# jeremy29tien/robosuite-benchmark

Hardware: AMD Instinct MI355X
Metric: SAC grad-steps/sec (batch=256, 1e6 buffer) at 1/2/4/8 GPU (higher is better)
Workload: dtype f32

## Files before the change

### robosuite_benchmark_amd/csrc/sac_trainer.hip

```cpp
#include "sac_common.h"

#include <algorithm>
#include <cmath>
#include <cstdlib>
#include <chrono>
#include <cstring>
#include <mutex>
#include <vector>

namespace sac {

typedef float f32x4 __attribute__((ext_vector_type(4)));

constexpr int H = 256;
constexpr float LOG_SIG_MAX = 2.0f, LOG_SIG_MIN = -20.0f, TANH_EPS = 1e-6f;
constexpr float ADAM_B1 = 0.9f, ADAM_B2 = 0.999f, ADAM_EPS = 1e-8f;
constexpr float ADAM_1MB1 = (float)(1.0 - 0.9), ADAM_1MB2 = (float)(1.0 - 0.999);
constexpr int DIAG_TRACE_CAP = 4096;
constexpr int M_SAC = 0, M_TD3_CRITIC = 1, M_TD3_ACTOR = 2;
constexpr int RD = 4;

struct StepArg {
    long long step_now;
    long long adam_t;
// ... 47 lines not shown
    float *diag_dev;
    const float *eps1, *eps2;
};

struct DwLayer {
    const float *dYT, *XT;
    long long xt_off;
    float *P, *PT, *MT, *VT, *G;
    float *bias, *mb, *vb, *gb;
    float *TP, *Tbias;
    int N, K, ldp, ldt, nk, job0, xt_from_slot;
    float lr;
    int k_base, pad_;
};
constexpr int NDW = 12;
struct DwTable {
    const DwLayer *L;
    int job0[NDW];
    int njobs;
    const unsigned *abort;
};

#ifdef SAC_STAMPS
__device__ unsigned long long g_stamps[5 * 512 * 16];
#define STAMP(kid, i)                                                                              \
    do {                                                                                           \
        __builtin_amdgcn_sched_barrier(0);                                                         \
        if (threadIdx.x == 0 && blockIdx.x < 512) {                                                \
            g_stamps[((kid) * 512 + blockIdx.x) * 16 + (i)] = wall_clock64();                      \
        }                                                                                          \
        __builtin_amdgcn_sched_barrier(0);                                                         \
    } while (0)
#define STAMP_CLK(kid, i)                                                                          \
    do {                                                                                           \
        if (threadIdx.x == 0 && blockIdx.x < 512) g_stamps[((kid) * 512 + blockIdx.x) * 16 + (i)] = clock64(); \
    } while (0)
#else
#define STAMP(kid, i) do { } while (0)
#define STAMP_CLK(kid, i) do { } while (0)
#endif

__device__ __forceinline__ int lds_off(int row, int k, int KL) {
    return row * KL + ((((k >> 2) ^ (row & 15)) << 2) | (k & 3));
}
#define SB() __builtin_amdgcn_sched_barrier(0)
#define USE_FROM_HERE(x) asm volatile("" : "+v"(x))
__device__ __forceinline__ void lds_barrier() { asm volatile("s_waitcnt lgkmcnt(0)\n\ts_barrier" ::: "memory"); }
template <typename T>
__device__ __forceinline__ T sload(const T *p) {
    return *(const __attribute__((address_space(4))) T *)(uintptr_t)p;
}
__device__ __forceinline__ f32x4 ld4(const float *p) { return *reinterpret_cast<const f32x4 *>(p); }
__device__ __forceinline__ float ld1g(const float *p) { return *(const __attribute__((address_space(1))) float *)(uintptr_t)p; }
__device__ __forceinline__ void st1g(float *p, float v) {
    __hip_atomic_store((__attribute__((address_space(1))) float *)(uintptr_t)p, v, __ATOMIC_RELAXED, __HIP_MEMORY_SCOPE_AGENT);
}

template <int NBYTES>
__device__ __forceinline__ void kernarg_prefetch() {
    typedef const __attribute__((address_space(4))) int *kptr;
    kptr ka = (kptr)__builtin_amdgcn_kernarg_segment_ptr();
    constexpr int NL = (NBYTES + 63) / 64;
    static_assert(NL <= 16, "kernarg_prefetch: more than 16 lines");
    int x[16];
#pragma unroll
    for (int i = 0; i < 16; ++i) x[i] = ka[i < NL ? i * 16 : 0];
    asm volatile("" ::"s"(x[0]), "s"(x[1]), "s"(x[2]), "s"(x[3]), "s"(x[4]), "s"(x[5]), "s"(x[6]), "s"(x[7]), "s"(x[8]),
                 "s"(x[9]), "s"(x[10]), "s"(x[11]), "s"(x[12]), "s"(x[13]), "s"(x[14]), "s"(x[15]));
}

__device__ __forceinline__ AlphaStep alpha_step(const Ctl *ctl, const float *part_logpi, int NB, int B, float target_entropy,
                                                float lr, int auto_alpha, double bc1, double bc2s) {
    AlphaStep r;
    const float la = sload(&ctl->log_alpha), m0 = sload(&ctl->a_m), v0 = sload(&ctl->a_v);
    if (!auto_alpha) { r.alpha = 1.0f; r.alpha_loss = 0.0f; r.log_alpha = la; r.m = m0; r.v = v0; return r; }
    float sum = 0.f;
    for (int i = 0; i < NB; ++i) sum += sload(part_logpi + i);
    const float mean_lp = sum / (float)B + target_entropy;
    r.alpha_loss = -((la * mean_lp) + 0.0f);
    const float gr = -mean_lp;
    r.m = m0 + ADAM_1MB1 * (gr - m0);
    r.v = v0 * ADAM_B2 + ADAM_1MB2 * gr * gr;
    const float step_size = (float)((double)lr / bc1);
    const float denom = sqrtf(r.v) / (float)bc2s + 1e-8f;
    r.log_alpha = la + (-step_size * r.m) / denom;
    r.alpha = expf(r.log_alpha);
    return r;
}
__device__ __forceinline__ void st4(float *p, f32x4 v) { *reinterpret_cast<f32x4 *>(p) = v; }

template <int NT, int D = RD>
struct WRing {
    f32x4 b[D][NT];
    const float *wp[NT];
    __device__ __forceinline__ void init(const float *W, int ldw, int n_base, int n_stride, int s_off = 0) {
        const int lane = threadIdx.x & 63;
#pragma unroll
        for (int t = 0; t < NT; ++t)
            wp[t] = W + ((size_t)((n_base + t * n_stride) >> 4) * (ldw >> 4) + s_off) * 256 + 4 * lane;
    }
    __device__ __forceinline__ void fill_part(int KS, int u0, int u1, int lo = 0) {
#pragma unroll
        for (int u = 0; u < D; ++u)
            if (u >= u0 && u < u1 && u < KS && u >= lo) {
#pragma unroll
                for (int t = 0; t < NT; ++t) b[u][t] = ld4(wp[t] + 256 * u);
// ... 912 lines not shown
    }
#pragma unroll
    for (int o = 32; o > 0; o >>= 1) {
#pragma unroll
        for (int q = 0; q < NS; ++q) {
            sm[q] += __shfl_xor(sm[q], o); sq[q] += __shfl_xor(sq[q], o);
            mx[q] = fmaxf(mx[q], __shfl_xor(mx[q], o)); mn[q] = fminf(mn[q], __shfl_xor(mn[q], o));
        }
        lsum += __shfl_xor(lsum, o);
    }
    double *sh = reinterpret_cast<double *>(red);
    if (lane == 0) {
#pragma unroll
        for (int q = 0; q < NS; ++q) {
            sh[wave * 32 + q] = sm[q]; sh[wave * 32 + 6 + q] = sq[q]; sh[wave * 32 + 12 + q] = mx[q]; sh[wave * 32 + 18 + q] = mn[q];
        }
        sh[wave * 32 + 24] = lsum;
    }
    lds_barrier();
    float *const dlast = d.diag_dev;
    auto put = [&](int di, float v) {
        dlast[di] = v;
        if (loop_pos == 0) d.diag_first[di] = v;
        if (loop_pos < DIAG_TRACE_CAP) d.diag_trace[(size_t)loop_pos * SAC_DIAG_N + di] = v;
    };
    if (threadIdx.x < NS) {
        const int q = threadIdx.x;
        if ((q < 5) ? (sa.pad & 1) : (sa.pad & 2)) {
            double s = 0, s2 = 0, MX = -INFINITY, MN = INFINITY;
            for (int w = 0; w < 4; ++w) {
                s += sh[w * 32 + q]; s2 += sh[w * 32 + 6 + q];
                MX = fmax(MX, sh[w * 32 + 12 + q]); MN = fmin(MN, sh[w * 32 + 18 + q]);
            }
            const double cnt = (q < 5) ? (double)B : (double)B * d.A;
            const double mean = s / cnt;
            double var = s2 / cnt - mean * mean;
            if (var < 0) var = 0;
            const int base = (q < 3) ? SAC_D_Q1_MEAN + 4 * q : SAC_D_LOGPI_MEAN + 4 * (q - 3);
            put(base, (float)mean); put(base + 1, (float)sqrt(var)); put(base + 2, (float)MX); put(base + 3, (float)MN);
            if (q == 3) put(SAC_D_QF1_LOSS, (float)mean);
            if (q == 4) put(SAC_D_QF2_LOSS, (float)mean);
        }
    } else if (threadIdx.x == 64 && (sa.pad & 2)) {
        double s = 0;
        for (int w = 0; w < 4; ++w) s += sh[w * 32 + 24];
        put(SAC_D_POLICY_LOSS, (float)(-s / B));
    }
    if (sa.pad2 & 2u) {
        __syncthreads();
        if (threadIdx.x < SAC_DIAG_N) d.diag_last[threadIdx.x] = ld_sc1(d.diag_dev + threadIdx.x);
    }
}

__device__ __forceinline__ void dw_adam_body(const Dev &d, const DwTable &T, const float *__restrict__ S, const StepArg &sa,
                                             float *red, float *redb, float *trs, int vblock, unsigned aborted) {
    const int B = d.B;
    const int wave = threadIdx.x >> 6, lane = threadIdx.x & 63;
    const int r = lane & 15, g = lane >> 4;
    const Ctl *cp = d.ctl;
    float *const dlast = (sa.pad2 & 2u) ? d.diag_last : d.diag_dev;
    const bool keep_grad = (sa.pad2 & 2u) != 0;
    const int jb = vblock - 1;
    if (jb >= 0) {
        STAMP(4 - 2 * (sa.loop_pos & 1), 0);
        int li = 0;
#pragma unroll
        for (int q = 1; q < NDW; ++q) li = (jb >= T.job0[q]) ? q : li;
        union { DwLayer J; unsigned long long w[sizeof(DwLayer) / 8]; } ud;
        {
            const __attribute__((address_space(4))) unsigned long long *src =
                (const __attribute__((address_space(4))) unsigned long long *)(uintptr_t)(T.L + li);
#pragma unroll
            for (int q = 0; q < (int)(sizeof(DwLayer) / 8); ++q) ud.w[q] = src[q];
        }
        const DwLayer &J = ud.J;
#ifdef SAC_STAMPS
        { unsigned long long probe = ud.w[0]; asm volatile("" :: "s"(probe)); }
        STAMP(4, 3);
#endif
        const int jj = jb - J.job0;
        const int n0 = 16 * (jj / J.nk), k0 = J.k_base + 64 * (jj % J.nk);
        const int k_own = k0 + 16 * wave + r;
        const bool own_valid = k_own < J.K;
        const size_t ot = frag_off(k_own, n0 + 4 * g, J.ldt);
        const size_t tile_floats = (size_t)(B >> 4) * 256;
        const float *XT = (J.xt_from_slot ? S + J.xt_off : J.XT) + (size_t)(k0 >> 4) * tile_floats;
        const float *YT = J.dYT + (size_t)(n0 >> 4) * tile_floats;
        const int per = (B / 16) / 4;
        const int rem = (B / 16) - 4 * per;
        const int s0 = wave * per + (wave < rem ? wave : rem);
        const int s1 = s0 + per + (wave < rem ? 1 : 0);
        const float *yp = YT + 4 * lane;
        const float *xp = XT + 4 * lane;
        f32x4 acc[4] = {};
        float bsum = 0.f;
        const f32x4 zero4 = {0.f, 0.f, 0.f, 0.f};
        auto chunk_of = [&](int sq) { const int m = (sq < s1 - 1) ? sq : s1 - 1; return m > 0 ? m : 0; };
        int nv = (J.ldp - k0) >> 4;
        nv = nv > 4 ? 4 : (nv < 1 ? 1 : nv);
        size_t toff[4];
#pragma unroll
        for (int t = 0; t < 4; ++t) toff[t] = (size_t)(t < nv ? t : nv - 1) * tile_floats;
        f32x4 a[4], b[4][4];
#pragma unroll
        for (int u = 0; u < 4; ++u) {
            const int cq = chunk_of(s0 + u);
            a[u] = ld4(yp + 256 * cq);
#pragma unroll
            for (int t = 0; t < 4; ++t) b[u][t] = ld4(xp + toff[t] + 256 * cq);
        }
        f32x4 p4 = {0.f, 0.f, 0.f, 0.f}, m4 = p4, v4 = p4;
        if (own_valid) {
            p4 = ld4(J.PT + ot);
            m4 = ld4(J.MT + ot);
            v4 = ld4(J.VT + ot);
        }
        const double bc1 = sa.bc1, bc2sd = sa.bc2s;
        const bool polyak = (J.TP != nullptr) && (sa.step_now % d.period == 0);
        const bool tile_ok = (k0 + 16 * wave) < J.ldp;
        const size_t pblk = frag_off(n0, k0 + 16 * wave, J.ldp) + 4 * lane;
        f32x4 tp4 = {0.f, 0.f, 0.f, 0.f};
        if (polyak && tile_ok) tp4 = ld4(J.TP + pblk);
        float pb = 0.f, mbv = 0.f, vbv = 0.f, tbv = 0.f;
        const bool bias_lane = (k0 == 0) && threadIdx.x < 16 && (n0 + (int)threadIdx.x) < J.N;
        if (bias_lane) {
            const int n = n0 + threadIdx.x;
            pb = ld1g(J.bias + n); mbv = ld1g(J.mb + n); vbv = ld1g(J.vb + n);
            if (polyak) tbv = ld1g(J.Tbias + n);
        }
#ifdef SAC_STAMPS
        { float probe = a[0][0] + b[3][3][3]; asm volatile("" :: "v"(probe)); }
        STAMP(4, 4);
#endif
        for (int sI = s0; sI < s1; sI += 4) {
#pragma unroll
            for (int u = 0; u < 4; ++u) {
                const f32x4 au = (sI + u < s1) ? a[u] : zero4;
                bsum += (au[0] + au[1]) + (au[2] + au[3]);
#pragma unroll
                for (int i = 0; i < 4; ++i) {
#pragma unroll
                    for (int t = 0; t < 4; ++t)
                        acc[t] = __builtin_amdgcn_mfma_f32_16x16x4f32(au[i], b[u][t][i], acc[t], 0, 0, 0);
                }
            }
            if (sI + 4 < s1) {
#pragma unroll
                for (int u = 0; u < 4; ++u) {
                    const int cq = chunk_of(sI + 4 + u);
                    a[u] = ld4(yp + 256 * cq);
#pragma unroll
                    for (int t = 0; t < 4; ++t) b[u][t] = ld4(xp + toff[t] + 256 * cq);
                }
            }
        }
#pragma unroll
        for (int t = 0; t < 4; ++t) st4(red + ((wave * 4 + t) * 64 + lane) * 4, acc[t]);
        bsum += __shfl_xor(bsum, 16);
        bsum += __shfl_xor(bsum, 32);
        if (g == 0) redb[wave * 16 + r] = bsum;
        lds_barrier();
        STAMP(4, 1);
        const float step_size = (float)((double)J.lr / bc1), bc2s = (float)bc2sd;
        if (aborted) return;
        if (tile_ok) {
            f32x4 gsum = {0.f, 0.f, 0.f, 0.f};
#pragma unroll
            for (int w = 0; w < 4; ++w) gsum += ld4(red + ((w * 4 + wave) * 64 + lane) * 4);
            if (own_valid) {
#pragma unroll
                for (int i = 0; i < 4; ++i) {
                    const int n = n0 + 4 * g + i;
                    if (n < J.N) {
                        float p = p4[i], m = m4[i], v = v4[i];
                        adam_update(p, m, v, gsum[i], step_size, bc2s);
                        p4[i] = p; m4[i] = m; v4[i] = v;
                        if (J.G && keep_grad) st1g(J.G + frag_off(n, k_own, J.ldp), gsum[i]);
                    }
                }
                st4_sc1(J.PT + ot, p4);
                st4_sc1(J.MT + ot, m4);
                st4_sc1(J.VT + ot, v4);
            }
            float *tw = trs + wave * 256;
#pragma unroll
            for (int i = 0; i < 4; ++i) tw[(4 * g + i) * 16 + r] = p4[i];
            __builtin_amdgcn_fence(__ATOMIC_RELEASE, "wavefront");
            __builtin_amdgcn_wave_barrier();
            __builtin_amdgcn_fence(__ATOMIC_ACQUIRE, "wavefront");
            const f32x4 pf = ld4(tw + r * 16 + 4 * g);
            st4_sc1(J.P + pblk, pf);
            if (polyak) st4_sc1(J.TP + pblk, tp4 * (1.0f - d.tau) + pf * d.tau);
        }
        if (bias_lane) {
            const int n = n0 + threadIdx.x;
            const float gb = (redb[threadIdx.x] + redb[16 + threadIdx.x]) + (redb[32 + threadIdx.x] + redb[48 + threadIdx.x]);
            adam_update(pb, mbv, vbv, gb, step_size, bc2s);
            st1g(J.bias + n, pb); st1g(J.mb + n, mbv); st1g(J.vb + n, vbv);
            if (J.gb && keep_grad) st1g(J.gb + n, gb);
            if (polyak) st1g(J.Tbias + n, tbv * (1.0f - d.tau) + pb * d.tau);
        }
        STAMP(4 - 2 * (sa.loop_pos & 1), 2);
    } else if (aborted) {
        if (threadIdx.x == 0 && d.diag_last[31] == 0.f) { d.diag_last[30] = __builtin_bit_cast(float, sa.seq); d.diag_last[31] = 1.f; }
    } else if (d.algo == 1) {
        td3_diagnostics(d, sa, red);
    } else {
        STAMP(3, 0);
        const int loop_pos = sa.loop_pos;
        const int Bt = d.Bt;
        const int i_first = (threadIdx.x < Bt) ? (int)threadIdx.x : 0;
        float yv0 = d.y[i_first], q10 = d.q[i_first], q20 = d.q[(size_t)B + i_first], lp0 = d.logpi[i_first];
        float qa0 = d.q[2 * (size_t)B + i_first], qb0 = d.q[3 * (size_t)B + i_first];
        f32x4 mu0[4], ls0[4];
#pragma unroll
        for (int j = 0; j < 4; ++j) { mu0[j] = ld4(d.mu + (size_t)i_first * 16 + 4 * j); ls0[j] = ld4(d.ls + (size_t)i_first * 16 + 4 * j); }
        SB();
        const AlphaStep as = alpha_step(cp, d.part_logpi, d.NB, d.Bt, d.target_entropy, d.alpha_lr, d.auto_alpha, sa.bc1, sa.bc2s);
        const float alpha = as.alpha, alpha_loss = as.alpha_loss;
#ifdef SAC_STAMPS
        { float probe = alpha; asm volatile("" ::"v"(probe)); STAMP(3, 2); }
        { float probe = ls0[3][3] + yv0; asm volatile("" ::"v"(probe)); STAMP(3, 3); }
#endif
        float *panel = red;
        const int qd = threadIdx.x >> 4, pl = threadIdx.x & 15;
        double r_s = 0, r_s2 = 0;
        float r_mx = -INFINITY, r_mn = INFINITY;
        for (int i0 = 0; i0 < Bt; i0 += 256) {
            const int i = i0 + threadIdx.x;
            {
                const float e1 = q10 - yv0, e2 = q20 - yv0;
                const float qn = fminf(qa0, qb0);
                float s_mu = 0.f, s_mu2 = 0.f, s_ls = 0.f, s_ls2 = 0.f, mx_mu = -INFINITY, mn_mu = INFINITY, mx_ls = -INFINITY, mn_ls = INFINITY;
#pragma unroll
                for (int j = 0; j < 4; ++j)
#pragma unroll
                    for (int u = 0; u < 4; ++u)
                        if (4 * j + u < d.A) {
                            const float m_ = mu0[j][u], l_ = ls0[j][u];
                            s_mu += m_; s_mu2 += m_ * m_; mx_mu = fmaxf(mx_mu, m_); mn_mu = fminf(mn_mu, m_);
                            s_ls += l_; s_ls2 += l_ * l_; mx_ls = fmaxf(mx_ls, l_); mn_ls = fminf(mn_ls, l_);
                        }
                const float vals[16] = {q10, q20, yv0, lp0, e1 * e1, e2 * e2, lp0 - qn, alpha * lp0 - qn,
                                        s_mu, s_mu2, mx_mu, mn_mu, s_ls, s_ls2, mx_ls, mn_ls};
#pragma unroll
                for (int q = 0; q < 16; ++q) panel[q * 256 + threadIdx.x] = vals[q];
            }
            lds_barrier();
            const int nrow = (Bt - i0 < 256) ? Bt - i0 : 256;
// ... 12 lines not shown
                for (int j = 0; j < 4; ++j) { mu0[j] = ld4(d.mu + (size_t)n * 16 + 4 * j); ls0[j] = ld4(d.ls + (size_t)n * 16 + 4 * j); }
            }
        }
#pragma unroll
        for (int o = 8; o > 0; o >>= 1) {
            r_s += __shfl_xor(r_s, o); r_s2 += __shfl_xor(r_s2, o);
            r_mx = fmaxf(r_mx, __shfl_xor(r_mx, o)); r_mn = fminf(r_mn, __shfl_xor(r_mn, o));
        }
#ifdef SAC_STAMPS
        { float probe = (float)r_s; asm volatile("" ::"v"(probe)); STAMP(3, 4); }
#endif
        double *tot = reinterpret_cast<double *>(redb);
        if (pl == 0) { tot[qd * 4 + 0] = r_s; tot[qd * 4 + 1] = r_s2; tot[qd * 4 + 2] = r_mx; tot[qd * 4 + 3] = r_mn; }
        lds_barrier();
        STAMP(3, 5);
        if (threadIdx.x < NSTAT) {
            const int q = threadIdx.x;
            double s, s2, MX, MN;
            if (q < 4) { s = tot[q * 4]; s2 = tot[q * 4 + 1]; MX = tot[q * 4 + 2]; MN = tot[q * 4 + 3]; }
            else { const int b0 = 8 + 4 * (q - 4); s = tot[b0 * 4]; s2 = tot[(b0 + 1) * 4]; MX = tot[(b0 + 2) * 4 + 2]; MN = tot[(b0 + 3) * 4 + 3]; }
            const double cnt = (q < 4) ? (double)Bt : (double)Bt * d.A;
            const double mean = s / cnt;
            double var = s2 / cnt - mean * mean;
            if (var < 0) var = 0;
            const float o4[4] = {(float)mean, (float)sqrt(var), (float)MX, (float)MN};
            for (int u = 0; u < 4; ++u) {
                const int di = SAC_D_Q1_MEAN + 4 * q + u;
                dlast[di] = o4[u];
                if (loop_pos == 0) d.diag_first[di] = o4[u];
                if (loop_pos < DIAG_TRACE_CAP) d.diag_trace[(size_t)loop_pos * SAC_DIAG_N + di] = o4[u];
            }
        } else if (threadIdx.x >= 64 && threadIdx.x < 64 + 8) {
            const int q = threadIdx.x - 64;
            float v = 0.f;
            int di = SAC_D_QF1_LOSS + q;
            if (q < 4) {
                v = (float)(tot[(4 + q) * 4] / Bt);
            } else if (q == 4) {
                v = alpha; di = SAC_D_ALPHA;
                Ctl *cw = d.ctl;
                cw->log_alpha = as.log_alpha; cw->a_m = as.m; cw->a_v = as.v; cw->alpha = as.alpha;
                cw->alpha_loss = as.alpha_loss;
            }
            else if (q == 5) { v = alpha_loss; di = SAC_D_ALPHA_LOSS; }
            else { di = 30 + (q - 6); }
            dlast[di] = v;
            if (loop_pos == 0) d.diag_first[di] = v;
            if (loop_pos < DIAG_TRACE_CAP) d.diag_trace[(size_t)loop_pos * SAC_DIAG_N + di] = v;
        }
        STAMP(3, 1);
    }
}

__global__ __launch_bounds__(256) void k_dw_adam(Dev d, DwTable T, const float *__restrict__ S, StepArg sa) {
    kernarg_prefetch<sizeof(Dev) + sizeof(DwTable) + 8 + sizeof(StepArg)>();
    __shared__ __attribute__((aligned(16))) float red[4 * 4 * 64 * 4];
    __shared__ __attribute__((aligned(16))) float redb[4 * 16 * 2];
    __shared__ __attribute__((aligned(16))) float trs[4 * 256];
    const unsigned aborted = T.abort ? sload(T.abort) : 0u;
    dw_adam_body(d, T, S, sa, red, redb, trs, (int)blockIdx.x, aborted);
}

#include "sac_bwd8.h"
#include "sac_fused.h"
#include "sac_chain.h"
#include "sac_general.h"

}

using namespace sac;

struct sac_general;

struct sac_trainer {
    sac_config_t cfg{};
    int device = 0;
    hipStream_t stream = nullptr;
    int B = 0, Bt = 0, O = 0, A = 0, KP = 0, KQ = 0, NH = 0, NB = 0, SP = 4;
    Net net[6];
    int HP[2] = {256, 256}, HQ[2] = {256, 256};
    int algo = 0;
    int td3_period = 2;
    long long adam_t_pi = 0;
    DwTable dw_q{}, dw_q_tp{}, dw_pi{}, dw_none{};
    void (*fwd_b2)(Dev, const float *, SlotLayout, StepArg) = nullptr;
    void (*bwd2)(Dev, const float *, SlotLayout, StepArg, int) = nullptr;
    Dev dev{};
    DwTable dw{};
    DwLayer *d_dwl = nullptr;
    char *arena = nullptr;
    float *ws = nullptr; int64_t ws_floats = 0;
    float *ext_slot = nullptr; SlotLayout ext_layout{};
    float *d_eps = nullptr;
    float *d_diag = nullptr;
    Ctl *d_ctl = nullptr;
    void *h_stage = nullptr; size_t stage_bytes = 0;
    hipEvent_t ev[4] = {nullptr, nullptr, nullptr, nullptr};
    static constexpr int NLOOP_EV = 12;
    hipEvent_t ev_ready[NLOOP_EV] = {}, ev_done[NLOOP_EV] = {};
    float *h_diag = nullptr, *d_diag_host = nullptr;
    float last_ms[4] = {0, 0, 0, 0};
    bool loop_primed = false;
    bool gate_exempt = false;
    bool timing_pending = false;
    hipEvent_t ev_tm[3] = {nullptr, nullptr, nullptr};
    std::vector<float> h_policy;
    bool mirror_valid = false;
    size_t lds_bw = 0;
    bool fused = false;
    unsigned fused_seq = 0;
    unsigned fused_unchecked = 0;
    bool publish_diag = true;
    unsigned test_stall_at = 0;
    static constexpr int NPEND = 64;
    struct Pending { sac_buffer *buf; int64_t token; };
    Pending pend[NPEND];
    int pend_n = 0;
    int pend_head = 0;
    long long dev_steps = 0;
    hipEvent_t thr_ev[4] = {nullptr, nullptr, nullptr, nullptr};
    int fallbacks = 0;
    void (*abc)(Dev, const float *, SlotLayout, StepArg) = nullptr;
    size_t lds_abc = 0;
    int abc_grid = 0, abc_threads = 256;
    bool chain_bwd = false;
    unsigned *d_sync = nullptr; size_t sync_bytes = 0;
    void (*fwd_a)(Dev, const float *, SlotLayout, int) = nullptr;
    void (*fwd_b)(Dev, const float *, SlotLayout, StepArg) = nullptr;
    void (*bwd)(Dev, const float *, SlotLayout, StepArg, int) = nullptr;
    size_t lds_fa = 0, lds_fb = 0;
    bool chain = false, chain8 = false;
    bool bwd8 = false;
    void (*chaink)(Dev, const float *, SlotLayout, StepArg) = nullptr;
    size_t lds_chain = 0;
    long long n_train_steps_total = 0, adam_t = 0;
    sac_general *gen = nullptr;
};

#include "sac_general_host.h"

namespace {

void build_layers(Net &n, const int (*shape)[2], int nl) {
    long long off = 0, offt = 0;
    for (int l = 0; l < nl; ++l) {
        Layer &L = n.L[l];
        L.N = shape[l][0]; L.K = shape[l][1];
        L.Np = round_up(L.N, 16); L.Kp = round_up(L.K, 16);
        L.offW = off; off += (long long)L.Np * L.Kp;
        L.offB = off; off += L.Np;
        off = round_up64(off, 4);
        L.offWt = offt; offt += (long long)(L.Kp + 16) * L.Np;
    }
    n.nP = off; n.nPT = offt;
}

struct Arena {
    std::vector<std::pair<void **, size_t>> req;
    size_t total = 0;
    void reserve(void **p, size_t bytes) {
        req.emplace_back(p, total);
// ... 45 lines not shown
        const int nshift = (netid == SAC_NET_POLICY && l == 3) ? t->A : 0;
        const bool qin = (netid >= 1 && netid <= 4) && l == 0;
        for (int n = 0; n < f.N[l]; ++n)
            for (int k = 0; k < f.K[l]; ++k) fn(fi++, dl, n + nshift, (qin && k >= t->O) ? t->KP + (k - t->O) : k, false);
        for (int n = 0; n < f.N[l]; ++n) fn(fi++, dl, n + nshift, 0, true);
    }
}

int ensure_stage_t(sac_trainer *t, size_t bytes) {
    if (t->stage_bytes >= bytes) return 0;
    if (t->h_stage) SAC_HIP(hipHostFree(t->h_stage));
    t->h_stage = nullptr; t->stage_bytes = 0;
    SAC_HIP(hipHostMalloc(&t->h_stage, bytes, hipHostMallocDefault));
    t->stage_bytes = bytes;
    return 0;
}

struct FusedGate { std::mutex mu; hipEvent_t ev = nullptr; hipStream_t last = nullptr; int live = 0; };
FusedGate g_gate[64];

int launch_fused_abc(sac_trainer *t, const float *S, const SlotLayout &SL, StepArg &sa, unsigned extra_flags) {
    hipStream_t s = t->stream;
    sa.seq = ++t->fused_seq;
    sa.pad2 |= extra_flags | ((t->test_stall_at && sa.seq == t->test_stall_at) ? 1u : 0u);
    t->fused_unchecked += 1;
    FusedGate &G = g_gate[t->device & 63];
    std::lock_guard<std::mutex> lk(G.mu);
    const bool gate = G.live > 1 && !t->gate_exempt;
    if (gate && G.last && G.last != s) SAC_HIP(hipStreamWaitEvent(s, G.ev, 0));
    hipLaunchKernelGGL(t->abc, dim3(t->abc_grid), dim3(t->abc_threads), t->lds_abc, s, t->dev, S, SL, sa);
    if (gate) { SAC_HIP(hipEventRecord(G.ev, s)); G.last = s; }
    return 0;
}

int launch_step_td3(sac_trainer *t, const float *S, const SlotLayout &SL, int j, bool want_stats) {
    const Dev &d = t->dev;
    hipStream_t s = t->stream;
    const int NB = t->NB, SPv = t->SP;
    const bool pstep = (t->n_train_steps_total % t->td3_period) == 0;
    const bool actor = pstep || want_stats;
    const double tq = (double)(t->adam_t + 1), tp = (double)(t->adam_t_pi + 1);
    StepArg sq{t->n_train_steps_total, t->adam_t + 1, j, 1, 1.0 - std::pow(0.9, tq), std::sqrt(1.0 - std::pow(0.999, tq))};
    StepArg sp{t->n_train_steps_total, t->adam_t_pi + 1, j, 2, 1.0 - std::pow(0.9, tp), std::sqrt(1.0 - std::pow(0.999, tp))};
    sq.pad2 = sp.pad2 = t->publish_diag ? 2u : 0u;
    if (t->fused) {
        if (launch_fused_abc(t, S, SL, sq, actor ? 4u : 0u)) return -1;
    } else {
        hipLaunchKernelGGL(t->fwd_a, dim3(4 * SPv * NB), dim3(256), t->lds_fa, s, d, S, SL, actor ? 1 : 0);
        const unsigned g2 = 8u * (unsigned)((SPv * NB + 3) / 4);
        hipLaunchKernelGGL(t->fwd_b, dim3(g2), dim3(256), t->lds_fb, s, d, S, SL, sq);
        hipLaunchKernelGGL(t->bwd, dim3(g2), dim3(256), t->lds_bw, s, d, S, SL, sq, 0);
    }
    const DwTable &Tq = pstep ? t->dw_q_tp : t->dw_q;
    hipLaunchKernelGGL(k_dw_adam, dim3(Tq.njobs + 1), dim3(256), 0, s, d, Tq, S, sq);
    if (actor) {
        hipLaunchKernelGGL(t->fwd_b2, dim3(SPv * NB), dim3(256), t->lds_fb, s, d, S, SL, sp);
        if (pstep) {
            hipLaunchKernelGGL(t->bwd2, dim3(SPv * NB), dim3(256), t->lds_bw, s, d, S, SL, sp, 0);
            hipLaunchKernelGGL(k_dw_adam, dim3(t->dw_pi.njobs + 1), dim3(256), 0, s, d, t->dw_pi, S, sp);
            t->adam_t_pi += 1;
        } else {
            hipLaunchKernelGGL(k_dw_adam, dim3(1), dim3(256), 0, s, d, t->dw_none, S, sp);
        }
    }
    SAC_HIP(hipGetLastError());
    t->n_train_steps_total += 1;
    t->adam_t += 1;
    return 0;
}


int launch_step(sac_trainer *t, const float *S, const SlotLayout &SL, int j, hipEvent_t *ev = nullptr, bool want_stats = false) {
    if (t->gen) return gen_launch_step(t, S, SL, j, want_stats);
    if (t->algo == 1) return launch_step_td3(t, S, SL, j, want_stats);
    const Dev &d = t->dev;
    hipStream_t s = t->stream;
    const int NB = t->NB;
    const double tt = (double)(t->adam_t + 1);
    StepArg sa{t->n_train_steps_total, t->adam_t + 1, j, 0, 1.0 - std::pow(0.9, tt), std::sqrt(1.0 - std::pow(0.999, tt))};
    sa.pad2 = t->publish_diag ? 2u : 0u;
    const int SPv = t->SP;
    if (ev) SAC_HIP(hipEventRecord(ev[0], s));
    if (t->fused) {
        if (launch_fused_abc(t, S, SL, sa, 0u)) return -1;
        if (ev) { SAC_HIP(hipEventRecord(ev[1], s)); SAC_HIP(hipEventRecord(ev[2], s)); SAC_HIP(hipEventRecord(ev[3], s)); }
    } else {
        if (t->chain) {
            hipLaunchKernelGGL(t->chaink, dim3(4 * NB), dim3(t->chain8 ? 512 : 256), t->lds_chain, s, d, S, SL, sa);
            if (ev) { SAC_HIP(hipEventRecord(ev[1], s)); SAC_HIP(hipEventRecord(ev[2], s)); }
        } else {
            hipLaunchKernelGGL(t->fwd_a, dim3(4 * SPv * NB), dim3(256), t->lds_fa, s, d, S, SL, 0);
            if (ev) SAC_HIP(hipEventRecord(ev[1], s));
            hipLaunchKernelGGL(t->fwd_b, dim3(4 * SPv * NB), dim3(256), t->lds_fb, s, d, S, SL, sa);
            if (ev) SAC_HIP(hipEventRecord(ev[2], s));
        }
        const int compact = (3 * SPv * NB <= 192) ? 1 : 0;
        hipLaunchKernelGGL(t->bwd, dim3(compact ? 4 * SPv * NB : 3 * SPv * NB), dim3(t->bwd8 ? 512 : 256), t->lds_bw, s, d, S, SL, sa, compact);
        if (ev) SAC_HIP(hipEventRecord(ev[3], s));
    }
    if (ev) SAC_HIP(hipEventRecord(ev[4], s));
    hipLaunchKernelGGL(k_dw_adam, dim3(t->dw.njobs + 1), dim3(256), 0, s, d, t->dw, S, sa);
    if (ev) { SAC_HIP(hipEventRecord(ev[5], s)); SAC_HIP(hipEventRecord(ev[6], s)); }
    SAC_HIP(hipGetLastError());
    t->n_train_steps_total += 1;
    t->adam_t += 1;
    return 0;
}

static int wait_trainer_stream(sac_trainer *t, hipEvent_t recorded = nullptr) {
    hipEvent_t e = recorded;
    if (!e) { e = t->ev[3]; SAC_HIP(hipEventRecord(e, t->stream)); }
    const auto spin_until = std::chrono::steady_clock::now() + std::chrono::milliseconds(2);
    hipError_t st;
    while ((st = hipEventQuery(e)) == hipErrorNotReady && std::chrono::steady_clock::now() < spin_until) { }
    if (st == hipSuccess) return 0;
    SAC_HIP(hipStreamSynchronize(t->stream));
    return 0;
}

static void set_abort_ptrs(sac_trainer *t, const unsigned *p) {
    t->dw.abort = p; t->dw_q.abort = p; t->dw_q_tp.abort = p; t->dw_pi.abort = p; t->dw_none.abort = p;
}

static int wait_event(hipEvent_t e) {
    const auto spin_until = std::chrono::steady_clock::now() + std::chrono::milliseconds(2);
    hipError_t st;
    while ((st = hipEventQuery(e)) == hipErrorNotReady && std::chrono::steady_clock::now() < spin_until) { }
    if (st == hipSuccess) return 0;
    if (st == hipErrorNotReady) (void)hipGetLastError();
    SAC_HIP(hipEventSynchronize(e));
    return 0;
}

int check_fused_abort(sac_trainer *t, unsigned *lost_out = nullptr) {
    const unsigned launched = t->fused_unchecked;
    t->fused_unchecked = 0;
    if (lost_out) *lost_out = 0;
    if (!t->fused || t->h_diag[SAC_DIAG_N + 31] == 0.f) { t->pend_n = 0; return 0; }
    unsigned first_bad = 0;
    memcpy(&first_bad, &t->h_diag[SAC_DIAG_N + 30], sizeof(unsigned));
    unsigned lost = t->fused_seq - first_bad + 1;
    if (lost > launched) lost = launched;
    t->n_train_steps_total -= lost;
    t->adam_t -= lost;
    t->fused = false;
    set_abort_ptrs(t, nullptr);
    if (t->algo == 1) {
        for (long long k = t->n_train_steps_total; k < t->n_train_steps_total + (long long)lost; ++k)
            if (k % t->td3_period == 0) t->adam_t_pi -= 1;
    }
    t->h_diag[SAC_DIAG_N + 30] = t->h_diag[SAC_DIAG_N + 31] = 0.f;
    SAC_HIP(hipMemsetAsync(t->d_sync, 0, t->sync_bytes, t->stream));
    SAC_HIP(hipStreamSynchronize(t->stream));
    if (!t->gate_exempt) {
// ... 209 lines not shown

    std::vector<DwLayer> hl;
    auto build_table = [&](DwTable &T, const std::vector<int> &nets, bool with_targets) {
        int job = 0, nl = 0;
        const size_t base = hl.size();
        for (int li = 0; li < NDW; ++li) T.job0[li] = 1 << 30;
        auto add_layer = [&](int netid, int l, const float *dYT, const float *XT, int from_slot, float lr, int part) {
            Net &n = t->net[netid];
            const Layer &L = n.L[l];
            const int nk_all = (L.Kp + 63) / 64;
            const bool has_tail = (l == 0) && (L.Kp % 64 != 0) && nk_all > 1;
            if (part == 1 && !has_tail) return;
            T.job0[nl++] = job;
            hl.emplace_back();
            DwLayer &J = hl.back();
            J.dYT = dYT; J.XT = XT; J.xt_from_slot = from_slot; J.xt_off = t->ext_layout.off_saT;
            J.P = n.P + L.offW; J.G = n.G + L.offW;
            J.PT = n.PT + L.offWt; J.MT = n.MT + L.offWt; J.VT = n.VT + L.offWt;
            J.bias = n.P + L.offB; J.mb = n.M + L.offB; J.vb = n.V + L.offB; J.gb = n.G + L.offB;
            J.TP = nullptr; J.Tbias = nullptr;
            const int tgt = (netid == 0) ? (td3 ? 5 : -1) : netid + 2;
            if (with_targets && tgt >= 0) {
                J.TP = t->net[tgt].P + L.offW;
                J.Tbias = t->net[tgt].P + L.offB;
            }
            J.ldp = L.Kp; J.ldt = L.Np; J.N = L.N; J.K = L.K; J.lr = lr;
            J.nk = (part == 1) ? 1 : (has_tail ? nk_all - 1 : nk_all);
            J.k_base = (part == 1) ? 64 * (nk_all - 1) : 0; J.pad_ = 0;
            J.job0 = job;
            job += (L.Np / 16) * J.nk;
        };
        const float *dY1[3] = {d.dPH2T, d.dQH2T, d.dQH2T + (size_t)H * B}, *X1[3] = {d.PH1T, d.QH1T, d.QH1T + (size_t)H * B};
        const float *dY0[3] = {d.dPH1T, d.dQH1T, d.dQH1T + (size_t)H * B};
        const float *dY2[3] = {d.dheadT, d.dq16T, d.dq16T + (size_t)16 * B}, *X2[3] = {d.PH2T, d.QH2T, d.QH2T + (size_t)H * B};
        const float lrs[3] = {cfg->policy_lr, cfg->qf_lr, cfg->qf_lr};
        for (int n : nets) add_layer(n, 1, dY1[n], X1[n], 0, lrs[n], 0);
        for (int n : nets) add_layer(n, 0, dY0[n], nullptr, 1, lrs[n], 0);
        for (int n : nets) add_layer(n, 2, dY2[n], X2[n], 0, lrs[n], 0);
        for (int n : nets) add_layer(n, 0, dY0[n], nullptr, 1, lrs[n], 1);
        T.njobs = job;
        T.L = t->d_dwl + base;
        T.abort = nullptr;
    };
    if (!td3) build_table(t->dw, {0, 1, 2}, true);
    else {
        build_table(t->dw_q, {1, 2}, false);
        build_table(t->dw_q_tp, {1, 2}, true);
        build_table(t->dw_pi, {0}, true);
        for (int li = 0; li < NDW; ++li) t->dw_none.job0[li] = 1 << 30;
        t->dw_none.njobs = 0; t->dw_none.L = t->d_dwl; t->dw_none.abort = nullptr;
        t->dw = t->dw_q;
    }
    SAC_HIP(hipMemcpyAsync(t->d_dwl, hl.data(), sizeof(DwLayer) * hl.size(), hipMemcpyHostToDevice, s));
    SAC_HIP(hipStreamSynchronize(s));

    const int KL0q = round_up(t->KQ, 64);
    const int nth = t->NH / 16;
    const int sw = 64 * (4 / t->SP);
    t->lds_fa = sizeof(float) * (size_t)(RB * KL0q + RB * H + RB * sw + 4 * nth * 256);
    t->lds_fb = sizeof(float) * (size_t)(RB * KL0q + RB * H + RB * sw + 1024 + (t->SP == 4 ? H * WLD : 0));
    t->lds_bw = sizeof(float) * (size_t)(RB * 64 + RB * H);
    SAC_REQUIRE(t->lds_fa <= 160 * 1024 - 512, "observation too wide for the LDS row-block budget (obs_dim=%d)", t->O);
    int wide_min = 16 * RD0 + 1;
    if (const char *e = getenv("SAC_WIDE_MIN_KQ")) wide_min = atoi(e);
    const bool wide = t->KQ >= wide_min;
#define SAC_PICK(SPV)                                                                                      \
    do {                                                                                                   \
        t->fwd_a = (nth == 1) ? (wide ? &k_fwd_a<1, true, SPV> : &k_fwd_a<1, false, SPV>)                   \
                              : (wide ? &k_fwd_a<2, true, SPV> : &k_fwd_a<2, false, SPV>);                  \
        t->fwd_b = (nth == 1) ? (wide ? &k_fwd_b<1, true, SPV> : &k_fwd_b<1, false, SPV>)                   \
                              : (wide ? &k_fwd_b<2, true, SPV> : &k_fwd_b<2, false, SPV>);                  \
        t->bwd = (nth == 1) ? &k_bwd<1, SPV> : &k_bwd<2, SPV>;                                             \
    } while (0)
#define TD3_PICK(SPV)                                                                                      \
    do {                                                                                                   \
        t->fwd_a = wide ? &k_fwd_a<1, true, SPV, M_TD3_CRITIC> : &k_fwd_a<1, false, SPV, M_TD3_CRITIC>;     \
        t->fwd_b = wide ? &k_fwd_b<1, true, SPV, M_TD3_CRITIC> : &k_fwd_b<1, false, SPV, M_TD3_CRITIC>;     \
        t->fwd_b2 = wide ? &k_fwd_b<1, true, SPV, M_TD3_ACTOR> : &k_fwd_b<1, false, SPV, M_TD3_ACTOR>;      \
        t->bwd = &k_bwd<1, SPV, M_TD3_CRITIC>;                                                             \
        t->bwd2 = &k_bwd<1, SPV, M_TD3_ACTOR>;                                                             \
    } while (0)
    if (!td3) {
        if (t->SP == 4) SAC_PICK(4);
        else if (t->SP == 2) SAC_PICK(2);
        else SAC_PICK(1);
    } else {
        if (t->SP == 4) TD3_PICK(4);
        else if (t->SP == 2) TD3_PICK(2);
        else TD3_PICK(1);
    }
#undef SAC_PICK
#undef TD3_PICK
    {
        int cus = 0;
        SAC_HIP(hipDeviceGetAttribute(&cus, hipDeviceAttributeMultiprocessorCount, t->device));
        const char *e = getenv("SAC_FUSED");
        t->lds_abc = sizeof(float) * (size_t)(RB * KL0q + RB * H + RB * 64 + FUSED_RED + H * WLD);
        t->fused = t->SP == 4 && t->NB <= 16 && 16 * t->NB <= cus && t->lds_abc <= 160 * 1024 - 512 && !(e && atoi(e) == 0);
        if (const char *ts = getenv("SAC_FUSED_TEST_STALL")) t->test_stall_at = (unsigned)atoi(ts);
        if (td3) t->abc = wide ? &k_abc<1, true, M_TD3_CRITIC> : &k_abc<1, false, M_TD3_CRITIC>;
        else t->abc = (nth == 1) ? (wide ? &k_abc<1, true> : &k_abc<1, false>) : (wide ? &k_abc<2, true> : &k_abc<2, false>);
        t->abc_grid = 16 * t->NB; t->abc_threads = 256;
        if (t->fused) {
            SAC_HIP(hipFuncSetAttribute(reinterpret_cast<const void *>(t->abc), hipFuncAttributeMaxDynamicSharedMemorySize,
                                        (int)t->lds_abc));
            set_abort_ptrs(t, d.abort_flag);
// ... 816 lines not shown
```

Measured before the change: 37680.

## Split dW GEMM by output tile per wave with LDS-shared dY in dw_adam

Adds a WAVE_TILE variant of the weight-gradient + Adam kernel. Each wave now owns one 16-column output tile and covers the whole batch, with dY fragments exchanged through LDS. This removes the cross-wave partial-sum reduction through LDS and the serial chunk loop, and issues all global loads up front, unconditionally, through global address-space loads. It is selected for B<=256 unless SAC_DW_TILE=0, and it assumes B/16 chunks fit within four per wave, which holds only at small batch.

Measured after the change: 38220 (median of 6 runs). No clear change (+1.4%).

```diff
diff --git a/robosuite_benchmark_amd/csrc/sac_trainer.hip b/robosuite_benchmark_amd/csrc/sac_trainer.hip
--- a/robosuite_benchmark_amd/csrc/sac_trainer.hip
+++ b/robosuite_benchmark_amd/csrc/sac_trainer.hip
@@ -123,6 +123,7 @@
 }
 __device__ __forceinline__ f32x4 ld4(const float *p) { return *reinterpret_cast<const f32x4 *>(p); }
 __device__ __forceinline__ float ld1g(const float *p) { return *(const __attribute__((address_space(1))) float *)(uintptr_t)p; }
+__device__ __forceinline__ f32x4 ld4g(const float *p) { return *(const __attribute__((address_space(1))) f32x4 *)(uintptr_t)p; }
 __device__ __forceinline__ void st1g(float *p, float v) {
     __hip_atomic_store((__attribute__((address_space(1))) float *)(uintptr_t)p, v, __ATOMIC_RELAXED, __HIP_MEMORY_SCOPE_AGENT);
 }
@@ -1141,6 +1142,7 @@
     }
 }
 
+template <bool WAVE_TILE>
 __device__ __forceinline__ void dw_adam_body(const Dev &d, const DwTable &T, const float *__restrict__ S, const StepArg &sa,
                                              float *red, float *redb, float *trs, int vblock, unsigned aborted) {
     const int B = d.B;
@@ -1177,29 +1179,47 @@
         const float *YT = J.dYT + (size_t)(n0 >> 4) * tile_floats;
         const int per = (B / 16) / 4;
         const int rem = (B / 16) - 4 * per;
-        const int s0 = wave * per + (wave < rem ? wave : rem);
-        const int s1 = s0 + per + (wave < rem ? 1 : 0);
+        auto q_s0 = [&](int q) { return q * per + (q < rem ? q : rem); };
+        auto q_s1 = [&](int q) { return q_s0(q) + per + (q < rem ? 1 : 0); };
+        const int s0 = q_s0(wave), s1 = q_s1(wave);
         const float *yp = YT + 4 * lane;
         const float *xp = XT + 4 * lane;
         f32x4 acc[4] = {};
         float bsum = 0.f;
         const f32x4 zero4 = {0.f, 0.f, 0.f, 0.f};
-        auto chunk_of = [&](int sq) { const int m = (sq < s1 - 1) ? sq : s1 - 1; return m > 0 ? m : 0; };
+        auto chunk_in = [](int sq, int e1) { const int m = (sq < e1 - 1) ? sq : e1 - 1; return m > 0 ? m : 0; };
+        auto chunk_of = [&](int sq) { return chunk_in(sq, s1); };
         int nv = (J.ldp - k0) >> 4;
         nv = nv > 4 ? 4 : (nv < 1 ? 1 : nv);
         size_t toff[4];
 #pragma unroll
         for (int t = 0; t < 4; ++t) toff[t] = (size_t)(t < nv ? t : nv - 1) * tile_floats;
         f32x4 a[4], b[4][4];
-#pragma unroll
-        for (int u = 0; u < 4; ++u) {
-            const int cq = chunk_of(s0 + u);
-            a[u] = ld4(yp + 256 * cq);
-#pragma unroll
-            for (int t = 0; t < 4; ++t) b[u][t] = ld4(xp + toff[t] + 256 * cq);
+        f32x4 xb[4][4];
+        if constexpr (WAVE_TILE) {
+#pragma unroll
+            for (int u = 0; u < 4; ++u) a[u] = ld4g(yp + 256 * chunk_of(s0 + u));
+            const float *xw = xp + toff[wave];
+#pragma unroll
+            for (int u = 0; u < 4; ++u) {
+#pragma unroll
+                for (int q = 0; q < 4; ++q) xb[q][u] = ld4g(xw + 256 * chunk_in(q_s0(q) + u, q_s1(q)));
+            }
+        } else {
+#pragma unroll
+            for (int u = 0; u < 4; ++u) {
+                const int cq = chunk_of(s0 + u);
+                a[u] = ld4(yp + 256 * cq);
+#pragma unroll
+                for (int t = 0; t < 4; ++t) b[u][t] = ld4(xp + toff[t] + 256 * cq);
+            }
         }
         f32x4 p4 = {0.f, 0.f, 0.f, 0.f}, m4 = p4, v4 = p4;
-        if (own_valid) {
+        if constexpr (WAVE_TILE) {
+            const size_t oq = own_valid ? ot : 0;
+            const f32x4 pl = ld4g(J.PT + oq), ml = ld4g(J.MT + oq), vl = ld4g(J.VT + oq);
+            if (own_valid) { p4 = pl; m4 = ml; v4 = vl; }
+        } else if (own_valid) {
             p4 = ld4(J.PT + ot);
             m4 = ld4(J.MT + ot);
             v4 = ld4(J.VT + ot);
@@ -1209,7 +1229,7 @@
         const bool tile_ok = (k0 + 16 * wave) < J.ldp;
         const size_t pblk = frag_off(n0, k0 + 16 * wave, J.ldp) + 4 * lane;
         f32x4 tp4 = {0.f, 0.f, 0.f, 0.f};
-        if (polyak && tile_ok) tp4 = ld4(J.TP + pblk);
+        if (polyak && tile_ok) tp4 = WAVE_TILE ? ld4g(J.TP + pblk) : ld4(J.TP + pblk);
         float pb = 0.f, mbv = 0.f, vbv = 0.f, tbv = 0.f;
         const bool bias_lane = (k0 == 0) && threadIdx.x < 16 && (n0 + (int)threadIdx.x) < J.N;
         if (bias_lane) {
@@ -1217,45 +1237,83 @@
             pb = ld1g(J.bias + n); mbv = ld1g(J.mb + n); vbv = ld1g(J.vb + n);
             if (polyak) tbv = ld1g(J.Tbias + n);
         }
-#ifdef SAC_STAMPS
-        { float probe = a[0][0] + b[3][3][3]; asm volatile("" :: "v"(probe)); }
-        STAMP(4, 4);
-#endif
-        for (int sI = s0; sI < s1; sI += 4) {
+        float step_size = (float)((double)J.lr / bc1);
+        const float bc2s = (float)bc2sd;
+        f32x4 gsum = {0.f, 0.f, 0.f, 0.f};
+        float gb = 0.f;
+        if constexpr (WAVE_TILE) {
+#pragma unroll
+            for (int u = 0; u < 4; ++u) st4(red + ((wave * 4 + u) * 64 + lane) * 4, (s0 + u < s1) ? a[u] : zero4);
+            USE_FROM_HERE(step_size);
+            lds_barrier();
+            f32x4 accq[4] = {};
+            float bq[4] = {0.f, 0.f, 0.f, 0.f};
 #pragma unroll
             for (int u = 0; u < 4; ++u) {
-                const f32x4 au = (sI + u < s1) ? a[u] : zero4;
-                bsum += (au[0] + au[1]) + (au[2] + au[3]);
-#pragma unroll
-                for (int i = 0; i < 4; ++i) {
-#pragma unroll
-                    for (int t = 0; t < 4; ++t)
-                        acc[t] = __builtin_amdgcn_mfma_f32_16x16x4f32(au[i], b[u][t][i], acc[t], 0, 0, 0);
+#pragma unroll
+                for (int q = 0; q < 4; ++q) {
+                    const f32x4 au = ld4(red + ((q * 4 + u) * 64 + lane) * 4);
+                    bq[q] += (au[0] + au[1]) + (au[2] + au[3]);
+#pragma unroll
+                    for (int i = 0; i < 4; ++i) accq[q] = __builtin_amdgcn_mfma_f32_16x16x4f32(au[i], xb[q][u][i], accq[q], 0, 0, 0);
                 }
             }
-            if (sI + 4 < s1) {
+#ifdef SAC_STAMPS
+            { float probe = accq[3][3]; asm volatile("" :: "v"(probe)); }
+            STAMP(4, 4);
+#endif
+#pragma unroll
+            for (int q = 0; q < 4; ++q) gsum += accq[q];
+            if (k0 == 0 && wave == 0) {
+#pragma unroll
+                for (int q = 0; q < 4; ++q) { bq[q] += __shfl_xor(bq[q], 16); bq[q] += __shfl_xor(bq[q], 32); }
+                gb = (bq[0] + bq[1]) + (bq[2] + bq[3]);
+            }
+            __builtin_amdgcn_s_waitcnt(0x0F70);
+            STAMP(4, 1);
+        } else {
+#ifdef SAC_STAMPS
+            { float probe = a[0][0] + b[3][3][3]; asm volatile("" :: "v"(probe)); }
+            STAMP(4, 4);
+#endif
+            for (int sI = s0; sI < s1; sI += 4) {
 #pragma unroll
                 for (int u = 0; u < 4; ++u) {
-                    const int cq = chunk_of(sI + 4 + u);
-                    a[u] = ld4(yp + 256 * cq);
-#pragma unroll
-                    for (int t = 0; t < 4; ++t) b[u][t] = ld4(xp + toff[t] + 256 * cq);
+                    const f32x4 au = (sI + u < s1) ? a[u] : zero4;
+                    bsum += (au[0] + au[1]) + (au[2] + au[3]);
+#pragma unroll
+                    for (int i = 0; i < 4; ++i) {
+#pragma unroll
+                        for (int t = 0; t < 4; ++t)
+                            acc[t] = __builtin_amdgcn_mfma_f32_16x16x4f32(au[i], b[u][t][i], acc[t], 0, 0, 0);
+                    }
+                }
+                if (sI + 4 < s1) {
+#pragma unroll
+                    for (int u = 0; u < 4; ++u) {
+                        const int cq = chunk_of(sI + 4 + u);
+                        a[u] = ld4(yp + 256 * cq);
+#pragma unroll
+                        for (int t = 0; t < 4; ++t) b[u][t] = ld4(xp + toff[t] + 256 * cq);
+                    }
                 }
             }
-        }
-#pragma unroll
-        for (int t = 0; t < 4; ++t) st4(red + ((wave * 4 + t) * 64 + lane) * 4, acc[t]);
-        bsum += __shfl_xor(bsum, 16);
-        bsum += __shfl_xor(bsum, 32);
-        if (g == 0) redb[wave * 16 + r] = bsum;
-        lds_barrier();
-        STAMP(4, 1);
-        const float step_size = (float)((double)J.lr / bc1), bc2s = (float)bc2sd;
+#pragma unroll
+            for (int t = 0; t < 4; ++t) st4(red + ((wave * 4 + t) * 64 + lane) * 4, acc[t]);
+            bsum += __shfl_xor(bsum, 16);
+            bsum += __shfl_xor(bsum, 32);
+            if (g == 0) redb[wave * 16 + r] = bsum;
+            lds_barrier();
+            STAMP(4, 1);
+            if (tile_ok) {
+#pragma unroll
+                for (int w = 0; w < 4; ++w) gsum += ld4(red + ((w * 4 + wave) * 64 + lane) * 4);
+            }
+            if (bias_lane)
+                gb = (redb[threadIdx.x] + redb[16 + threadIdx.x]) + (redb[32 + threadIdx.x] + redb[48 + threadIdx.x]);
+        }
         if (aborted) return;
         if (tile_ok) {
-            f32x4 gsum = {0.f, 0.f, 0.f, 0.f};
-#pragma unroll
-            for (int w = 0; w < 4; ++w) gsum += ld4(red + ((w * 4 + wave) * 64 + lane) * 4);
             if (own_valid) {
 #pragma unroll
                 for (int i = 0; i < 4; ++i) {
@@ -1283,7 +1341,6 @@
         }
         if (bias_lane) {
             const int n = n0 + threadIdx.x;
-            const float gb = (redb[threadIdx.x] + redb[16 + threadIdx.x]) + (redb[32 + threadIdx.x] + redb[48 + threadIdx.x]);
             adam_update(pb, mbv, vbv, gb, step_size, bc2s);
             st1g(J.bias + n, pb); st1g(J.mb + n, mbv); st1g(J.vb + n, vbv);
             if (J.gb && keep_grad) st1g(J.gb + n, gb);
@@ -1402,13 +1459,14 @@
     }
 }
 
+template <bool WAVE_TILE>
 __global__ __launch_bounds__(256) void k_dw_adam(Dev d, DwTable T, const float *__restrict__ S, StepArg sa) {
     kernarg_prefetch<sizeof(Dev) + sizeof(DwTable) + 8 + sizeof(StepArg)>();
     __shared__ __attribute__((aligned(16))) float red[4 * 4 * 64 * 4];
     __shared__ __attribute__((aligned(16))) float redb[4 * 16 * 2];
     __shared__ __attribute__((aligned(16))) float trs[4 * 256];
     const unsigned aborted = T.abort ? sload(T.abort) : 0u;
-    dw_adam_body(d, T, S, sa, red, redb, trs, (int)blockIdx.x, aborted);
+    dw_adam_body<WAVE_TILE>(d, T, S, sa, red, redb, trs, (int)blockIdx.x, aborted);
 }
 
 #include "sac_bwd8.h"
@@ -1457,6 +1515,7 @@
     std::vector<float> h_policy;
     bool mirror_valid = false;
     size_t lds_bw = 0;
+    void (*dw_adam)(Dev, DwTable, const float *, StepArg) = nullptr;
     bool fused = false;
     unsigned fused_seq = 0;
     unsigned fused_unchecked = 0;
@@ -1608,15 +1667,15 @@
         hipLaunchKernelGGL(t->bwd, dim3(g2), dim3(256), t->lds_bw, s, d, S, SL, sq, 0);
     }
     const DwTable &Tq = pstep ? t->dw_q_tp : t->dw_q;
-    hipLaunchKernelGGL(k_dw_adam, dim3(Tq.njobs + 1), dim3(256), 0, s, d, Tq, S, sq);
+    hipLaunchKernelGGL(t->dw_adam, dim3(Tq.njobs + 1), dim3(256), 0, s, d, Tq, S, sq);
     if (actor) {
         hipLaunchKernelGGL(t->fwd_b2, dim3(SPv * NB), dim3(256), t->lds_fb, s, d, S, SL, sp);
         if (pstep) {
             hipLaunchKernelGGL(t->bwd2, dim3(SPv * NB), dim3(256), t->lds_bw, s, d, S, SL, sp, 0);
-            hipLaunchKernelGGL(k_dw_adam, dim3(t->dw_pi.njobs + 1), dim3(256), 0, s, d, t->dw_pi, S, sp);
+            hipLaunchKernelGGL(t->dw_adam, dim3(t->dw_pi.njobs + 1), dim3(256), 0, s, d, t->dw_pi, S, sp);
             t->adam_t_pi += 1;
         } else {
-            hipLaunchKernelGGL(k_dw_adam, dim3(1), dim3(256), 0, s, d, t->dw_none, S, sp);
+            hipLaunchKernelGGL(t->dw_adam, dim3(1), dim3(256), 0, s, d, t->dw_none, S, sp);
         }
     }
     SAC_HIP(hipGetLastError());
@@ -1655,7 +1714,7 @@
         if (ev) SAC_HIP(hipEventRecord(ev[3], s));
     }
     if (ev) SAC_HIP(hipEventRecord(ev[4], s));
-    hipLaunchKernelGGL(k_dw_adam, dim3(t->dw.njobs + 1), dim3(256), 0, s, d, t->dw, S, sa);
+    hipLaunchKernelGGL(t->dw_adam, dim3(t->dw.njobs + 1), dim3(256), 0, s, d, t->dw, S, sa);
     if (ev) { SAC_HIP(hipEventRecord(ev[5], s)); SAC_HIP(hipEventRecord(ev[6], s)); }
     SAC_HIP(hipGetLastError());
     t->n_train_steps_total += 1;
@@ -1971,6 +2030,10 @@
         t->dw = t->dw_q;
     }
     SAC_HIP(hipMemcpyAsync(t->d_dwl, hl.data(), sizeof(DwLayer) * hl.size(), hipMemcpyHostToDevice, s));
+    {
+        const char *e = getenv("SAC_DW_TILE");
+        t->dw_adam = (B <= 256 && !(e && atoi(e) == 0)) ? &k_dw_adam<true> : &k_dw_adam<false>;
+    }
     SAC_HIP(hipStreamSynchronize(s));
 
     const int KL0q = round_up(t->KQ, 64);
```
